# envoyproxy/ai-gateway

Hardware: AMD Instinct MI355X
Metric: req/sec (whole node) + p50 added latency, OpenAI chat/completions 4k-token body (higher is better)
Workload: dtype bf16; 1 GPU; model=aigw standalone: OpenAI /v1/chat/completions -> mock upstream (examples/basic), global_batch=128, seq_len=4096, parallelism=dp1, front=fast, cpu_affinity=numa node 1 (128 cpus)

## Files before the change

csrc/admission.hip:

```cpp

#include <hip/hip_runtime.h>

#include <atomic>
#include <cstdint>
#include <cstdio>
#include <cstring>
#include <mutex>
#include <vector>

#include "bpe_kernels.cuh"
#include "cache_kernels.cuh"

namespace aigw_fast {

namespace {

__global__ void excl_scan_kernel(const int32_t* __restrict__ in, int n,
                                 int32_t* __restrict__ excl,
                                 int32_t* __restrict__ total) {
  __shared__ int32_t wave_sum[4];
  __shared__ int32_t carry_s;
  if (threadIdx.x == 0) carry_s = 0;
  __syncthreads();
  int lane = (int)threadIdx.x & 63;
  int wave = (int)threadIdx.x >> 6;
  for (int base = 0; base < n; base += 256) {
    int i = base + (int)threadIdx.x;
    int32_t orig = (i < n) ? in[i] : 0;
    int32_t v = orig;
    for (int off = 1; off < 64; off <<= 1) {
      int32_t t = __shfl_up(v, off);
      if (lane >= off) v += t;
    }
    if (lane == 63) wave_sum[wave] = v;
    __syncthreads();
    int32_t wave_off = 0;
    for (int w = 0; w < wave; ++w) wave_off += wave_sum[w];
    if (i < n) excl[i] = carry_s + wave_off + v - orig;
    int32_t chunk_total =
        wave_sum[0] + wave_sum[1] + wave_sum[2] + wave_sum[3];
    __syncthreads();
    if (threadIdx.x == 0) carry_s += chunk_total;
    __syncthreads();
  }
  if (threadIdx.x == 0) *total = carry_s;
}

__global__ void f32_to_bf16_kernel(const float* __restrict__ in,
                                   bf16* __restrict__ out, int n) {
  int i = blockIdx.x * blockDim.x + threadIdx.x;
  if (i < n) out[i] = (bf16)in[i];
}

__global__ void tok_flags_kernel(const int32_t* __restrict__ out_ids, int n,
                                 uint8_t* __restrict__ flags) {
  int i = blockIdx.x * blockDim.x + threadIdx.x;
  if (i < n) flags[i] = out_ids[i] >= 0;
}

__global__ void meanpool_tokens_kernel(
    const int32_t* __restrict__ ids, const int32_t* __restrict__ ghead,
    const int32_t* __restrict__ req_excl, const int32_t* __restrict__ counts,
    int n_req, const bf16* __restrict__ emb, int dim, int P,
    float* __restrict__ out, int32_t* __restrict__ cnt) {
  constexpr int STAGE = 128;
  __shared__ int32_t tok_ids[STAGE];
  int r = blockIdx.x;
  int p = blockIdx.y;
  if (r >= n_req) return;
  int dim2 = dim >> 1;
  int col2 = threadIdx.x;
  int s = req_excl[r], c = counts[r];
  int chunk = (c + P - 1) / P;
  int j0 = p * chunk;
  int j1 = j0 + chunk;
  if (j1 > c) j1 = c;
  const uint32_t* emb2 = reinterpret_cast<const uint32_t*>(emb);
  float acc_lo = 0.f, acc_hi = 0.f;
  int n = 0;
  for (int base = j0; base < j1; base += STAGE) {
    if (threadIdx.x < STAGE && base + (int)threadIdx.x < j1)
      tok_ids[threadIdx.x] = ids[ghead[s + base + threadIdx.x]];
    __syncthreads();
    int here = j1 - base < STAGE ? j1 - base : STAGE;
    if (col2 < dim2) {
      for (int q = 0; q < here; ++q) {
        int tok = tok_ids[q];
        if (tok < 0) continue;
        uint32_t v = emb2[(long long)tok * dim2 + col2];
        bf16 lo, hi;
        uint16_t vlo = (uint16_t)(v & 0xffffu), vhi = (uint16_t)(v >> 16);
        memcpy(&lo, &vlo, 2);
        memcpy(&hi, &vhi, 2);
        acc_lo += __bfloat162float(lo);
        acc_hi += __bfloat162float(hi);
        ++n;
      }
    }
    __syncthreads();
  }
  if (col2 < dim2 && n) {
    atomicAdd(&out[(long long)r * dim + 2 * col2], acc_lo);
    atomicAdd(&out[(long long)r * dim + 2 * col2 + 1], acc_hi);
    if (col2 == 0) atomicAdd(&cnt[r], n);
  }
}

__global__ void park_pending_kernel(const bf16* __restrict__ q,
                                    const int32_t* __restrict__ slots,
                                    int n_req, int dim,
                                    bf16* __restrict__ pending) {
  int r = blockIdx.x;
  int col = threadIdx.x;
  if (r >= n_req || col >= dim) return;
  int slot = slots[r];
  if (slot < 0) return;
  pending[(size_t)slot * dim + col] = q[(size_t)r * dim + col];
}

__global__ void bf16_to_fp8_kernel(const bf16* __restrict__ in,
                                   uint8_t* __restrict__ out, int n) {
  int i = (blockIdx.x * blockDim.x + threadIdx.x) * 2;
  if (i >= n) return;
  float a = (float)in[i];
  float b = (i + 1 < n) ? (float)in[i + 1] : 0.f;
  int packed = __builtin_amdgcn_cvt_pk_fp8_f32(a, b, 0, false);
  out[i] = (uint8_t)(packed & 0xff);
  if (i + 1 < n) out[i + 1] = (uint8_t)((packed >> 8) & 0xff);
}

#define HIP_OK(expr)                                                   \
  do {                                                                 \
    hipError_t _e = (expr);                                            \
    if (_e != hipSuccess) {                                            \
      fprintf(stderr, "aigw admission: %s failed: %s\n", #expr,        \
              hipGetErrorString(_e));                                  \
      return false;                                                    \
    }                                                                  \
  } while (0)

}

class GpuAdmissionDirect {
 public:
  static constexpr int kSets = 2;

  struct BatchSet {
    hipStream_t stream{};
    hipEvent_t event{};
    char* h_bytes = nullptr;
    int64_t* h_off = nullptr;
    int32_t* h_counts = nullptr;
    unsigned long long* h_best = nullptr;
    int32_t* h_slots = nullptr;
    uint8_t* d_bytes = nullptr;
    int64_t* d_off = nullptr;
    uint8_t* d_flags = nullptr;
    uint8_t* d_gflags = nullptr;
    int32_t* d_blk = nullptr;
    int32_t* d_excl = nullptr;
    int32_t* d_totals = nullptr;
    int32_t* d_seg_start = nullptr;
    int32_t* d_seg_req = nullptr;
    int32_t* d_ghead = nullptr;
    int32_t* d_out_ids = nullptr;
    int32_t* d_counts = nullptr;
    int32_t* d_req_excl = nullptr;
    float* d_pool = nullptr;
    int32_t* d_poolcnt = nullptr;
    bf16* d_poolbf = nullptr;
    float* d_gout = nullptr;
    bf16* d_q = nullptr;
    uint8_t* d_q8 = nullptr;
    unsigned long long* d_best = nullptr;
    int32_t* d_slots = nullptr;
    long long rows_in_flight = 0;
  };

  bool init(const long long* htab_keys, const int32_t* htab_rank, int htab_n,
            size_t max_bytes, int max_req, int device) {
    int count = 0;
    if (hipGetDeviceCount(&count) != hipSuccess || count == 0) return false;
    device_ = device >= 0 && device < count ? device : 0;
    HIP_OK(hipSetDevice(device_));
    max_bytes_ = max_bytes;
    max_req_ = max_req;
    htab_mask_ = htab_n - 1;
    HIP_OK(hipMalloc(&d_htab_keys_, sizeof(long long) * htab_n));
    HIP_OK(hipMalloc(&d_htab_rank_, sizeof(int32_t) * htab_n));
    HIP_OK(hipMemcpy(d_htab_keys_, htab_keys, sizeof(long long) * htab_n,
                     hipMemcpyHostToDevice));
    HIP_OK(hipMemcpy(d_htab_rank_, htab_rank, sizeof(int32_t) * htab_n,
                     hipMemcpyHostToDevice));
    int max_blocks = (int)((max_bytes + 255) / 256);
    for (int s = 0; s < kSets; ++s) {
      BatchSet& b = sets_[s];
      HIP_OK(hipStreamCreateWithFlags(&b.stream, hipStreamNonBlocking));
      HIP_OK(hipEventCreateWithFlags(
          &b.event, hipEventDisableTiming | hipEventBlockingSync));
      HIP_OK(hipHostMalloc(&b.h_bytes, max_bytes, hipHostMallocDefault));
      HIP_OK(hipHostMalloc(&b.h_off, sizeof(int64_t) * (max_req + 1),
                           hipHostMallocDefault));
      HIP_OK(hipHostMalloc(&b.h_counts, sizeof(int32_t) * max_req,
                           hipHostMallocDefault));
      HIP_OK(hipMalloc(&b.d_bytes, max_bytes));
      HIP_OK(hipMalloc(&b.d_off, sizeof(int64_t) * (max_req + 1)));
      HIP_OK(hipMalloc(&b.d_flags, max_bytes));
      HIP_OK(hipMalloc(&b.d_gflags, max_bytes));
      HIP_OK(hipMalloc(&b.d_blk, sizeof(int32_t) * max_blocks));
      HIP_OK(hipMalloc(&b.d_excl, sizeof(int32_t) * max_blocks));
      HIP_OK(hipMalloc(&b.d_totals, sizeof(int32_t) * 2));
      HIP_OK(hipMalloc(&b.d_seg_start, sizeof(int32_t) * max_bytes));
      HIP_OK(hipMalloc(&b.d_seg_req, sizeof(int32_t) * max_bytes));
      HIP_OK(hipMalloc(&b.d_ghead, sizeof(int32_t) * max_bytes));
      HIP_OK(hipMalloc(&b.d_out_ids, sizeof(int32_t) * max_bytes));
      HIP_OK(hipMalloc(&b.d_counts, sizeof(int32_t) * max_req));
      HIP_OK(hipMalloc(&b.d_req_excl, sizeof(int32_t) * (max_req + 1)));
    }
    ready_ = true;
    return true;
  }

  bool count(const char* bytes, size_t n, const int64_t* offsets, int n_req,
             int32_t* counts_out) {
    if (!submit(0, bytes, n, offsets, n_req, nullptr)) return false;
    return wait_set(0, n_req, counts_out, nullptr, nullptr);
  }

  bool submit(int s, const char* bytes, size_t n, const int64_t* offsets,
              int n_req, const int32_t* pending_slots) {
    if (!ready_ || n == 0 || n_req == 0 || n > max_bytes_ || n_req > max_req_)
      return false;
    BatchSet& b = sets_[s];
    HIP_OK(hipSetDevice(device_));
    if (bytes != nullptr) memcpy(b.h_bytes, bytes, n);
    memcpy(b.h_off, offsets, sizeof(int64_t) * (size_t)n_req);
    hipStream_t st = b.stream;
    HIP_OK(hipMemcpyAsync(b.d_bytes, b.h_bytes, n, hipMemcpyHostToDevice, st));
    HIP_OK(hipMemcpyAsync(b.d_off, b.h_off, sizeof(int64_t) * (size_t)n_req,
                          hipMemcpyHostToDevice, st));
    int blocks = (int)((n + 255) / 256);
    hipLaunchKernelGGL(seg_flags_count_kernel, dim3(blocks), dim3(256), 0, st,
                       b.d_bytes, (int)n, b.d_off, n_req, b.d_flags, b.d_blk,
                       b.d_counts);
    hipLaunchKernelGGL(excl_scan_kernel, dim3(1), dim3(256), 0, st,
                       b.d_blk, blocks, b.d_excl, b.d_totals);
    hipLaunchKernelGGL(seg_write_kernel, dim3(blocks), dim3(256), 0, st,
                       b.d_flags, (int)n, b.d_excl, b.d_off, n_req,
                       b.d_seg_start, b.d_seg_req);
    hipLaunchKernelGGL(group_flags_count_kernel, dim3(blocks), dim3(256), 0,
                       st, b.d_seg_start, b.d_seg_req, b.d_totals, b.d_off,
                       (int)n, b.d_gflags, b.d_blk);
    hipLaunchKernelGGL(excl_scan_kernel, dim3(1), dim3(256), 0, st,
                       b.d_blk, blocks, b.d_excl, b.d_totals + 1);
    hipLaunchKernelGGL(flag_compact_write_kernel, dim3(blocks), dim3(256), 0,
                       st, b.d_gflags, (int)n, b.d_excl, b.d_ghead);
    bool want_cache = pending_slots != nullptr && cache_on_;
    if (want_cache)
      HIP_OK(hipMemsetAsync(b.d_out_ids, 0xFF, sizeof(int32_t) * n, st));
    long long group_bound = (long long)n / 32 + n_req + 1;
    constexpr int kBpeBlock = 512;
    constexpr int kGroupsPerBlock = kBpeBlock / 64;
    int blocks2 = (int)((group_bound + kGroupsPerBlock - 1) / kGroupsPerBlock);
    hipLaunchKernelGGL(bpe_encode_grouped_dev_kernel, dim3(blocks2),
                       dim3(kBpeBlock), 0, st, b.d_bytes, b.d_seg_start, b.d_seg_req,
                       b.d_totals, (int)n, b.d_ghead, b.d_totals + 1,
                       d_htab_keys_, d_htab_rank_, htab_mask_, b.d_out_ids,
                       b.d_counts);
    if (want_cache) {
      if (!submit_cache(b, n, n_req, pending_slots)) return false;
    }
    HIP_OK(hipMemcpyAsync(b.h_counts, b.d_counts, sizeof(int32_t) * n_req,
                          hipMemcpyDeviceToHost, st));
    HIP_OK(hipEventRecord(b.event, st));
    return true;
  }

  bool wait_set(int s, int n_req, int32_t* counts_out, int32_t* rows_out,
                float* scores_out) {
    BatchSet& b = sets_[s];
    HIP_OK(hipEventSynchronize(b.event));
    memcpy(counts_out, b.h_counts, sizeof(int32_t) * (size_t)n_req);
    if (rows_out != nullptr && scores_out != nullptr) {
      long long rows_now = b.rows_in_flight;
      for (int i = 0; i < n_req; ++i) {
        rows_out[i] = -1;
        scores_out[i] = 0.f;
        if (rows_now > 0) {
          unsigned long long u = b.h_best[i];
          unsigned hi = (unsigned)(u >> 32);
          unsigned bits = (hi >= 0x80000000u) ? (hi ^ 0x80000000u) : ~hi;
          float score;
          memcpy(&score, &bits, 4);
          if (score >= threshold_) {
            rows_out[i] = (int32_t)(u & 0xFFFFFFFFu);
            scores_out[i] = score;
          }
        }
      }
    }
    return true;
  }


  char* staging(int s) { return sets_[s].h_bytes; }

  bool init_cache(const uint16_t* emb, int vocab, const uint16_t* proj,
                  int dim, long long capacity, float threshold,
                  int pending_cap, bool fp8) {
    if (!ready_ || dim != 384) return false;
    HIP_OK(hipSetDevice(device_));
    dim_ = dim;
    cap_ = capacity;
    threshold_ = threshold;
    vocab_ = vocab;
    pending_cap_ = pending_cap;
    fp8_ = fp8;
    HIP_OK(hipMalloc(&d_emb_, sizeof(bf16) * (size_t)vocab * dim));
    HIP_OK(hipMemcpy(d_emb_, emb, sizeof(bf16) * (size_t)vocab * dim,
                     hipMemcpyHostToDevice));
    HIP_OK(hipMalloc(&d_proj_, sizeof(bf16) * (size_t)dim * dim));
    HIP_OK(hipMemcpy(d_proj_, proj, sizeof(bf16) * (size_t)dim * dim,
                     hipMemcpyHostToDevice));
    size_t elt = fp8 ? 1 : sizeof(bf16);
    HIP_OK(hipMalloc(&d_index_, elt * (size_t)capacity * dim));
    HIP_OK(hipMemset(d_index_, 0, elt * (size_t)capacity * dim));
    HIP_OK(hipMalloc(&d_pending_, sizeof(bf16) * (size_t)pending_cap * dim));
    HIP_OK(hipStreamCreateWithFlags(&insert_stream_, hipStreamNonBlocking));
    for (int s = 0; s < kSets; ++s) {
      BatchSet& b = sets_[s];
      HIP_OK(hipMalloc(&b.d_pool, sizeof(float) * (size_t)max_req_ * dim));
      HIP_OK(hipMalloc(&b.d_poolcnt, sizeof(int32_t) * max_req_));
      HIP_OK(hipMalloc(&b.d_poolbf, sizeof(bf16) * (size_t)max_req_ * dim));
      HIP_OK(hipMalloc(&b.d_gout, sizeof(float) * (size_t)max_req_ * dim));
      HIP_OK(hipMalloc(&b.d_q, sizeof(bf16) * (size_t)max_req_ * dim));
      if (fp8) HIP_OK(hipMalloc(&b.d_q8, (size_t)max_req_ * dim));
      HIP_OK(hipMalloc(&b.d_best, sizeof(unsigned long long) * max_req_));
      HIP_OK(hipHostMalloc(&b.h_best, sizeof(unsigned long long) * max_req_,
                           hipHostMallocDefault));
// ... 48 lines not shown
                       b.d_q, b.d_slots, n_req, dim, d_pending_);
    long long rows_now = rows_visible_.load(std::memory_order_acquire);
    b.rows_in_flight = rows_now;
    if (rows_now > 0) {
      HIP_OK(hipMemsetAsync(b.d_best, 0, sizeof(unsigned long long) * n_req, st));
      constexpr int ROWTILES = 16;
      long long blocks = (rows_now + 64 * ROWTILES - 1) / (64 * ROWTILES);
      if (fp8_) {
        hipLaunchKernelGGL(bf16_to_fp8_kernel,
                           dim3((n_req * dim / 2 + 255) / 256), dim3(256), 0,
                           st, b.d_q, b.d_q8, n_req * dim);
        constexpr size_t L8 = 128 * (12 * 32 + 16) + 128 * 8;
        (void)hipFuncSetAttribute(
            reinterpret_cast<const void*>(
                &cache_topk_fp8_lds_kernel_t<12, ROWTILES>),
            hipFuncAttributeMaxDynamicSharedMemorySize, 160 * 1024);
        for (int q0 = 0; q0 < n_req; q0 += 128) {
          int kq = (n_req - q0) < 128 ? (n_req - q0) : 128;
          hipLaunchKernelGGL((cache_topk_fp8_lds_kernel_t<12, ROWTILES>),
                             dim3((unsigned)blocks), dim3(256), L8, st,
                             (const uint8_t*)d_index_, rows_now,
                             b.d_q8 + (size_t)q0 * dim, kq, dim, b.d_best + q0);
        }
      } else {
        constexpr size_t L = 128 * (12 * 32 + 8) * sizeof(bf16) + 128 * 8;
        (void)hipFuncSetAttribute(
            reinterpret_cast<const void*>(&cache_topk_lds_kernel_t<12, ROWTILES>),
            hipFuncAttributeMaxDynamicSharedMemorySize, 160 * 1024);
        for (int q0 = 0; q0 < n_req; q0 += 128) {
          int kq = (n_req - q0) < 128 ? (n_req - q0) : 128;
          hipLaunchKernelGGL((cache_topk_lds_kernel_t<12, ROWTILES>),
                             dim3((unsigned)blocks), dim3(256), L, st,
                             (const bf16*)d_index_, rows_now,
                             b.d_q + (size_t)q0 * dim, kq, dim, b.d_best + q0);
        }
      }
      HIP_OK(hipMemcpyAsync(b.h_best, b.d_best,
                            sizeof(unsigned long long) * n_req,
                            hipMemcpyDeviceToHost, st));
    }
    return true;
  }

  bool count_lookup(const char* bytes, size_t n, const int64_t* offsets,
                    int n_req, int32_t* counts_out,
                    const int32_t* pending_slots, int32_t* rows_out,
                    float* scores_out) {
    if (!cache_on_) return false;
    if (!submit(0, bytes, n, offsets, n_req, pending_slots)) return false;
    return wait_set(0, n_req, counts_out, rows_out, scores_out);
  }

  long long cache_insert(int pending_slot) {
    if (!cache_on_ || pending_slot < 0 || pending_slot >= pending_cap_)
      return -1;
    long long row = head_;
    head_ = (head_ + 1) % cap_;
    if (fp8_) {
      hipLaunchKernelGGL(bf16_to_fp8_kernel, dim3((dim_ / 2 + 255) / 256),
                         dim3(256), 0, insert_stream_,
                         d_pending_ + (size_t)pending_slot * dim_,
                         (uint8_t*)d_index_ + (size_t)row * dim_, dim_);
      if (hipGetLastError() != hipSuccess) return -1;
    } else {
      hipError_t e = hipMemcpyAsync(
          (bf16*)d_index_ + (size_t)row * dim_,
          d_pending_ + (size_t)pending_slot * dim_, sizeof(bf16) * dim_,
          hipMemcpyDeviceToDevice, insert_stream_);
      if (e != hipSuccess) return -1;
    }
    long long vis = rows_visible_.load(std::memory_order_relaxed);
    long long want = row + 1 > vis ? row + 1 : vis;
    if (want > cap_) want = cap_;
    rows_visible_.store(want, std::memory_order_release);
    return row;
  }

  ~GpuAdmissionDirect() {
    if (!ready_) return;
    for (int s = 0; s < kSets; ++s) {
      BatchSet& b = sets_[s];
      (void)hipStreamDestroy(b.stream);
      (void)hipEventDestroy(b.event);
      (void)hipHostFree(b.h_bytes);
      (void)hipHostFree(b.h_off);
      (void)hipHostFree(b.h_counts);
      (void)hipHostFree(b.h_best);
      (void)hipHostFree(b.h_slots);
      for (void* p : {(void*)b.d_bytes, (void*)b.d_off, (void*)b.d_flags,
                      (void*)b.d_gflags, (void*)b.d_blk, (void*)b.d_excl,
                      (void*)b.d_totals, (void*)b.d_seg_start,
                      (void*)b.d_seg_req, (void*)b.d_ghead,
                      (void*)b.d_out_ids, (void*)b.d_counts, (void*)b.d_pool,
                      (void*)b.d_poolcnt, (void*)b.d_poolbf, (void*)b.d_gout,
                      (void*)b.d_q, (void*)b.d_q8, (void*)b.d_best,
                      (void*)b.d_slots})
        (void)hipFree(p);
    }
    if (cache_on_) {
      (void)hipStreamDestroy(insert_stream_);
      for (void* p : {(void*)d_emb_, (void*)d_proj_, (void*)d_index_,
                      (void*)d_pending_})
        (void)hipFree(p);
    }
    for (void* p : {(void*)d_htab_keys_, (void*)d_htab_rank_})
      (void)hipFree(p);
  }

  bool ready() const { return ready_; }

 private:
  bool ready_ = false;
  bool cache_on_ = false;
  int device_ = 0;
  int dim_ = 0;
  int vocab_ = 0;
  int pending_cap_ = 0;
  long long cap_ = 0;
  long long head_ = 0;
  std::atomic<long long> rows_visible_{0};
  float threshold_ = 0.f;
  bool fp8_ = false;
  bf16* d_emb_ = nullptr;
  bf16* d_proj_ = nullptr;
  void* d_index_ = nullptr;
  bf16* d_pending_ = nullptr;
  hipStream_t insert_stream_{};
  size_t max_bytes_ = 0;
  int max_req_ = 0;
  int htab_mask_ = 0;
  long long* d_htab_keys_ = nullptr;
  int32_t* d_htab_rank_ = nullptr;
  BatchSet sets_[kSets];
};

GpuAdmissionDirect* admission_create(const long long* htab_keys,
                                     const int32_t* htab_rank, int htab_n,
                                     size_t max_bytes, int max_req, int device) {
  auto* a = new GpuAdmissionDirect();
  if (!a->init(htab_keys, htab_rank, htab_n, max_bytes, max_req, device)) {
    delete a;
    return nullptr;
  }
  return a;
}

bool admission_count(GpuAdmissionDirect* a, const char* bytes, size_t n,
                     const int64_t* offsets, int n_req, int32_t* counts_out) {
  return a->count(bytes, n, offsets, n_req, counts_out);
}

void admission_destroy(GpuAdmissionDirect* a) { delete a; }

bool admission_init_cache(GpuAdmissionDirect* a, const uint16_t* emb, int vocab,
                          const uint16_t* proj, int dim, long long capacity,
                          float threshold, int pending_cap, bool fp8) {
  return a->init_cache(emb, vocab, proj, dim, capacity, threshold, pending_cap,
                       fp8);
}

bool admission_count_lookup(GpuAdmissionDirect* a, const char* bytes, size_t n,
                            const int64_t* offsets, int n_req,
                            int32_t* counts_out, const int32_t* pending_slots,
                            int32_t* rows_out, float* scores_out) {
  return a->count_lookup(bytes, n, offsets, n_req, counts_out, pending_slots,
                         rows_out, scores_out);
}

long long admission_cache_insert(GpuAdmissionDirect* a, int pending_slot) {
  return a->cache_insert(pending_slot);
}

bool admission_submit(GpuAdmissionDirect* a, int set, const char* bytes,
                      size_t n, const int64_t* offsets, int n_req,
                      const int32_t* pending_slots) {
  return a->submit(set, bytes, n, offsets, n_req, pending_slots);
}

bool admission_wait(GpuAdmissionDirect* a, int set, int n_req,
                    int32_t* counts_out, int32_t* rows_out,
                    float* scores_out) {
  return a->wait_set(set, n_req, counts_out, rows_out, scores_out);
}

char* admission_staging(GpuAdmissionDirect* a, int set) {
  return a->staging(set);
}

}
```

csrc/aigw_fast_module.cpp:

```cpp

#include <pybind11/pybind11.h>
#include <pybind11/stl.h>

#include <cstdint>
#include <stdexcept>
#include <string>
#include <vector>

#include "fastpath.h"

namespace py = pybind11;
using namespace aigw_fast;

namespace aigw_fast {

GpuAdmissionDirect* admission_create(const long long* htab_keys,
                                     const int32_t* htab_rank, int htab_n,
                                     size_t max_bytes, int max_req, int device);
bool admission_count(GpuAdmissionDirect* a, const char* bytes, size_t n,
                     const int64_t* offsets, int n_req, int32_t* counts_out);
void admission_destroy(GpuAdmissionDirect* a);
bool admission_init_cache(GpuAdmissionDirect* a, const uint16_t* emb, int vocab,
                          const uint16_t* proj, int dim, long long capacity,
                          float threshold, int pending_cap, bool fp8);
bool admission_count_lookup(GpuAdmissionDirect* a, const char* bytes, size_t n,
                            const int64_t* offsets, int n_req,
                            int32_t* counts_out, const int32_t* pending_slots,
                            int32_t* rows_out, float* scores_out);
long long admission_cache_insert(GpuAdmissionDirect* a, int pending_slot);

}

namespace {

class AdmissionProbe {
 public:
  AdmissionProbe(py::buffer htab_keys, py::buffer htab_rank, size_t max_bytes,
                 int max_req, int device)
      : max_bytes_(max_bytes), max_req_(max_req) {
    py::buffer_info ki = htab_keys.request();
    py::buffer_info ri = htab_rank.request();
    if (ki.itemsize != 8 || ri.itemsize != 4)
      throw std::runtime_error("htab_keys must be int64, htab_rank int32");
    if (ki.size != ri.size || ki.size <= 0 || (ki.size & (ki.size - 1)) != 0)
      throw std::runtime_error("htab arrays must share a power-of-two length");
    if (max_bytes == 0 || max_req <= 0)
      throw std::runtime_error("max_bytes and max_req must be positive");
    adm_ = admission_create(static_cast<const long long*>(ki.ptr),
                            static_cast<const int32_t*>(ri.ptr), (int)ki.size,
                            max_bytes, max_req, device);
    if (adm_ == nullptr) throw std::runtime_error("admission init failed");
  }
  AdmissionProbe(const AdmissionProbe&) = delete;
  AdmissionProbe& operator=(const AdmissionProbe&) = delete;
  ~AdmissionProbe() {
    if (adm_ != nullptr) admission_destroy(adm_);
  }

  void init_cache(py::buffer emb, py::buffer proj, long long capacity,
                  float threshold, int pending_cap, bool fp8) {
    constexpr int dim = 384;
    py::buffer_info ei = emb.request();
    py::buffer_info pi = proj.request();
    if (ei.itemsize != 2 || pi.itemsize != 2)
      throw std::runtime_error("emb/proj must be bf16 (uint16 view)");
    int vocab = (int)(ei.size / dim);
    if (vocab <= 0 || (long long)vocab * dim != ei.size ||
        pi.size != (long long)dim * dim)
      throw std::runtime_error("emb/proj shape mismatch");
    if (capacity <= 0 || pending_cap <= 0)
      throw std::runtime_error("capacity and pending_cap must be positive");
    if (cache_on_) throw std::runtime_error("cache already initialised");
    if (!admission_init_cache(adm_, static_cast<const uint16_t*>(ei.ptr), vocab,
                              static_cast<const uint16_t*>(pi.ptr), dim,
                              capacity, threshold, pending_cap, fp8))
      throw std::runtime_error("native cache init failed");
    pending_cap_ = pending_cap;
    cache_on_ = true;
  }

  std::vector<int32_t> count(const std::vector<std::string>& texts) {
    pack(texts);
    std::vector<int32_t> counts(texts.size(), 0);
    bool ok;
    {
      py::gil_scoped_release release;
      ok = admission_count(adm_, bytes_.data(), bytes_.size(), offs_.data(),
                           (int)texts.size(), counts.data());
    }
    if (!ok) throw std::runtime_error("admission_count failed");
    return counts;
  }

  py::tuple count_lookup(const std::vector<std::string>& texts) {
    if (!cache_on_) throw std::runtime_error("init_cache() first");
    if ((long long)texts.size() > pending_cap_)
      throw std::runtime_error("more texts than pending slots");
    pack(texts);
    size_t nt = texts.size();
    std::vector<int32_t> counts(nt, 0), rows(nt, -1), slots(nt);
    std::vector<float> scores(nt, 0.f);
    for (size_t i = 0; i < nt; ++i) slots[i] = (int32_t)i;
    bool ok;
    {
      py::gil_scoped_release release;
      ok = admission_count_lookup(adm_, bytes_.data(), bytes_.size(),
                                  offs_.data(), (int)nt, counts.data(),
                                  slots.data(), rows.data(), scores.data());
    }
    if (!ok) throw std::runtime_error("admission_count_lookup failed");
    return py::make_tuple(counts, rows, scores);
  }

  long long insert(int slot) {
    if (!cache_on_) throw std::runtime_error("init_cache() first");
    long long row = admission_cache_insert(adm_, slot);
    if (row < 0) throw std::runtime_error("cache insert failed");
    return row;
  }

 private:
  void pack(const std::vector<std::string>& texts) {
    if (texts.empty() || (long long)texts.size() > max_req_)
      throw std::runtime_error("text count out of range");
    bytes_.clear();
    offs_.clear();
    for (const auto& t : texts) {
      offs_.push_back((int64_t)bytes_.size());
      bytes_.append(t);
    }
    if (bytes_.empty() || bytes_.size() > max_bytes_)
      throw std::runtime_error("batch bytes out of range");
  }

  GpuAdmissionDirect* adm_ = nullptr;
  size_t max_bytes_;
  int max_req_;
  int pending_cap_ = 0;
  bool cache_on_ = false;
  std::string bytes_;
  std::vector<int64_t> offs_;
};

}

PYBIND11_MODULE(aigw_fast, m) {
  m.doc() = "aigw native data-plane fast path";

  py::class_<AdmissionProbe>(m, "AdmissionProbe")
      .def(py::init<py::buffer, py::buffer, size_t, int, int>(),
           py::arg("htab_keys"), py::arg("htab_rank"), py::arg("max_bytes"),
           py::arg("max_req"), py::arg("device") = 0)
      .def("init_cache", &AdmissionProbe::init_cache, py::arg("emb_u16"),
           py::arg("proj_u16"), py::arg("capacity"), py::arg("threshold"),
           py::arg("pending_cap"), py::arg("fp8"))
      .def("count", &AdmissionProbe::count, py::arg("texts"))
      .def("count_lookup", &AdmissionProbe::count_lookup, py::arg("texts"))
      .def("insert", &AdmissionProbe::insert, py::arg("slot"));

  py::class_<FastMock>(m, "FastMock")
      .def(py::init<>())
      .def("start", &FastMock::start, py::arg("host"), py::arg("response"))
      .def("stop", &FastMock::stop)
      .def("requests", &FastMock::requests);

  m.def(
      "run_load",
      [](const std::string& host, uint16_t port, const std::string& path,
         py::bytes body, int connections, int per_conn) {
        LoadResult r;
        {
          std::string b = body;
          py::gil_scoped_release release;
          r = run_load(host, port, path, b, connections, per_conn);
        }
        py::dict d;
        d["elapsed_s"] = r.elapsed_s;
        d["completed"] = r.completed;
        d["errors"] = r.errors;
        d["p50_ms"] = r.p50_ms;
        d["p99_ms"] = r.p99_ms;
        return d;
      },
      py::arg("host"), py::arg("port"), py::arg("path"), py::arg("body"),
      py::arg("connections"), py::arg("per_conn"),
      "closed-loop native load generator (threads, keep-alive)");

  m.def(
      "run_load_pool",
      [](const std::string& host, uint16_t port, const std::string& path,
         py::list bodies, int connections, int per_conn, bool capture_last) {
        std::vector<std::string> pool;
        for (auto b : bodies) pool.push_back(b.cast<py::bytes>());
        LoadResult r;
        {
          py::gil_scoped_release release;
          r = run_load_pool(host, port, path, pool, connections, per_conn,
                            capture_last);
        }
        py::dict d;
        d["elapsed_s"] = r.elapsed_s;
        d["completed"] = r.completed;
        d["errors"] = r.errors;
        d["p50_ms"] = r.p50_ms;
        d["p99_ms"] = r.p99_ms;
        if (capture_last) {
          py::list last;
          for (const auto& b : r.last_bodies) last.append(py::bytes(b));
          d["last_bodies"] = last;
        }
        return d;
      },
      py::arg("host"), py::arg("port"), py::arg("path"), py::arg("bodies"),
      py::arg("connections"), py::arg("per_conn"),
      py::arg("capture_last") = false,
      "run_load with a cycling body pool (semantic-cache hit mixes); "
      "capture_last also returns each connection's final response body");

  py::class_<FastServer>(m, "FastServer")
      .def(py::init<>())
      .def(
          "add_route",
          [](FastServer& s, const std::string& name, const std::string& model_match,
             int retries, bool has_costs, bool eligible, py::list backends) {
            FastRoute r;
            r.name = name;
            r.model_match = model_match;
            r.retries = retries;
            r.has_costs = has_costs;
            r.eligible = eligible;
            for (auto item : backends) {
              py::dict d = item.cast<py::dict>();
              FastBackend b;
              b.name = d["name"].cast<std::string>();
              b.host = d["host"].cast<std::string>();
              b.port = d["port"].cast<uint16_t>();
              if (d.contains("bearer")) b.bearer = d["bearer"].cast<std::string>();
              if (d.contains("api_key_file"))
                b.api_key_file = d["api_key_file"].cast<std::string>();
              if (d.contains("model_override"))
// ... 140 lines not shown
```

csrc/bpe_kernels.cuh:

```cuda
#pragma once

#include <hip/hip_runtime.h>

#include <climits>
#include <cstdint>

__device__ __forceinline__ int byte_class(uint8_t b) {
  if (b == ' ') return 0;
  if (b == '\t' || b == '\n' || b == '\r' || b == 0x0b || b == 0x0c) return 1;
  if (b >= '0' && b <= '9') return 2;
  if ((b >= 'A' && b <= 'Z') || (b >= 'a' && b <= 'z') || b >= 0x80) return 3;
  return 4;
}

__global__ void seg_flags_kernel(const uint8_t* __restrict__ bytes, int n,
                                 uint8_t* __restrict__ flags) {
  int i = blockIdx.x * blockDim.x + threadIdx.x;
  if (i >= n) return;
  uint8_t f;
  if (i == 0) {
    f = 1;
  } else {
    uint8_t b = bytes[i], p = bytes[i - 1];
    f = (b == ' ') || (byte_class(b) != byte_class(p) && p != ' ');
// ... 311 lines not shown

__global__ void group_head_flags_kernel(const int32_t* __restrict__ seg_start,
                                        const int32_t* __restrict__ seg_req,
                                        int n_segs,
                                        const int64_t* __restrict__ req_off,
                                        uint8_t* __restrict__ flags) {
  int i = blockIdx.x * blockDim.x + threadIdx.x;
  if (i >= n_segs) return;
  uint8_t f;
  if (i == 0 || seg_req[i] != seg_req[i - 1]) {
    f = 1;
  } else {
    long long off = req_off[seg_req[i]];
    f = ((seg_start[i] - off) >> 5) != ((seg_start[i - 1] - off) >> 5);
  }
  flags[i] = f;
}

__global__ void group_head_flags_dev_kernel(const int32_t* __restrict__ seg_start,
                                            const int32_t* __restrict__ seg_req,
                                            const int32_t* __restrict__ n_segs_dev,
                                            const int64_t* __restrict__ req_off,
                                            uint8_t* __restrict__ flags) {
  int i = blockIdx.x * blockDim.x + threadIdx.x;
  if (i >= *n_segs_dev) return;
  uint8_t f;
  if (i == 0 || seg_req[i] != seg_req[i - 1]) {
    f = 1;
  } else {
    long long off = req_off[seg_req[i]];
    f = ((seg_start[i] - off) >> 5) != ((seg_start[i - 1] - off) >> 5);
  }
  flags[i] = f;
}

__global__ void __launch_bounds__(256)
group_flags_count_kernel(const int32_t* __restrict__ seg_start,
                         const int32_t* __restrict__ seg_req,
                         const int32_t* __restrict__ n_segs_dev,
                         const int64_t* __restrict__ req_off, int n,
                         uint8_t* __restrict__ flags,
                         int32_t* __restrict__ blk_counts) {
  int i = blockIdx.x * 256 + threadIdx.x;
  bool f = false;
  if (i < n) {
    if (i < *n_segs_dev) {
      if (i == 0 || seg_req[i] != seg_req[i - 1]) {
        f = true;
      } else {
        long long off = req_off[seg_req[i]];
        f = ((seg_start[i] - off) >> 5) != ((seg_start[i - 1] - off) >> 5);
      }
    }
    flags[i] = f;
  }
  int cnt = block256_flag_count(f);
  if (threadIdx.x == 0) blk_counts[blockIdx.x] = cnt;
}

__global__ void flag_compact_write_kernel(const uint8_t* __restrict__ flags, int n,
                                          const int32_t* __restrict__ blk_excl,
                                          int32_t* __restrict__ out_idx) {
  __shared__ int wave_base[4];
  int i = blockIdx.x * blockDim.x + threadIdx.x;
  int lane = threadIdx.x & 63;
  int wave = threadIdx.x >> 6;
  bool f = (i < n) && flags[i];
  uint64_t ballot = __ballot(f);
  if (lane == 0) wave_base[wave] = __popcll(ballot);
  __syncthreads();
  if (threadIdx.x == 0) {
    int acc = 0;
    for (int w = 0; w < 4; ++w) {
      int c = wave_base[w];
      wave_base[w] = acc;
      acc += c;
    }
  }
  __syncthreads();
  if (!f) return;
  int pos_in_wave = __popcll(ballot & ((1ull << lane) - 1ull));
  out_idx[blk_excl[blockIdx.x] + wave_base[wave] + pos_in_wave] = i;
}
```

setup.py:

```python

import os

from setuptools import setup

os.environ.setdefault("PYTORCH_ROCM_ARCH", "gfx950")

import pybind11
from setuptools import Extension
from torch.utils.cpp_extension import BuildExtension, CUDAExtension

setup(
    name="aigw",
    version="0.1.0",
    packages=["aigw"],
    ext_modules=[
        CUDAExtension(
            name="aigw_hip",
            sources=["csrc/aigw_kernels.hip"],
            extra_compile_args={
                "cxx": ["-O3", "-std=c++17"],
                "nvcc": ["-O3", "-std=c++17", "--offload-arch=gfx950"],
            },
        ),
        Extension(
            name="aigw_native",
            sources=["csrc/aigw_native.cpp"],
            include_dirs=[pybind11.get_include()],
            extra_compile_args=["-O3", "-std=c++17"],
            language="c++",
        ),
        CUDAExtension(
            name="aigw_fast",
            sources=[
                "csrc/aigw_fast_module.cpp",
                "csrc/fastpath.cpp",
                "csrc/admission.hip",
            ],
            extra_compile_args={
                "cxx": ["-O3", "-std=c++17"],
                "nvcc": ["-O3", "-std=c++17", "--offload-arch=gfx950"],
            },
            extra_link_args=["-lpthread"],
        ),
    ],
    cmdclass={"build_ext": BuildExtension},
)
```

Baseline: 218,600 req/s.

## Fuse admission pre-tokenize kernels with last-block scans and single staged upload

Rewrites the GPU admission front end so each 256-thread block processes a 4096-byte granule instead of 256 bytes. The separate single-block exclusive-scan launches are folded into the flag/count kernels through a last-block-done ticket. Offsets and bytes now share one staging buffer, so a single H2D copy replaces two, with an optional zero-copy path that is off by default. This cuts kernel launches and per-batch overhead at the cost of atomic ticket synchronization and fewer, larger blocks. It also adds a pipelined count API and a build-flag hook.

```diff
diff --git a/csrc/admission.hip b/csrc/admission.hip
--- a/csrc/admission.hip
+++ b/csrc/admission.hip
@@ -10,6 +10,13 @@
 
 #include "bpe_kernels.cuh"
 #include "cache_kernels.cuh"
+
+#ifndef AIGW_ADM_FOLD_UPLOAD
+#define AIGW_ADM_FOLD_UPLOAD 0
+#endif
+#ifndef AIGW_ADM_FOLD_SCAN
+#define AIGW_ADM_FOLD_SCAN 1
+#endif
 
 namespace aigw_fast {
 
@@ -148,18 +155,20 @@
   struct BatchSet {
     hipStream_t stream{};
     hipEvent_t event{};
+    char* h_stage = nullptr;
+    uint8_t* d_stage = nullptr;
+    uint8_t* h_stage_dev = nullptr;
     char* h_bytes = nullptr;
-    int64_t* h_off = nullptr;
     int32_t* h_counts = nullptr;
     unsigned long long* h_best = nullptr;
     int32_t* h_slots = nullptr;
     uint8_t* d_bytes = nullptr;
-    int64_t* d_off = nullptr;
     uint8_t* d_flags = nullptr;
     uint8_t* d_gflags = nullptr;
     int32_t* d_blk = nullptr;
     int32_t* d_excl = nullptr;
     int32_t* d_totals = nullptr;
+    unsigned* d_tickets = nullptr;
     int32_t* d_seg_start = nullptr;
     int32_t* d_seg_req = nullptr;
     int32_t* d_ghead = nullptr;
@@ -193,29 +202,42 @@
     HIP_OK(hipMemcpy(d_htab_rank_, htab_rank, sizeof(int32_t) * htab_n,
                      hipMemcpyHostToDevice));
     int max_blocks = (int)((max_bytes + 255) / 256);
+    size_t padded = (max_bytes + kAdmGranule - 1) / kAdmGranule * kAdmGranule;
+    header_bytes_ = (sizeof(int64_t) * ((size_t)max_req + 1) + 255) / 256 * 256;
     for (int s = 0; s < kSets; ++s) {
       BatchSet& b = sets_[s];
       HIP_OK(hipStreamCreateWithFlags(&b.stream, hipStreamNonBlocking));
       HIP_OK(hipEventCreateWithFlags(
           &b.event, hipEventDisableTiming | hipEventBlockingSync));
-      HIP_OK(hipHostMalloc(&b.h_bytes, max_bytes, hipHostMallocDefault));
-      HIP_OK(hipHostMalloc(&b.h_off, sizeof(int64_t) * (max_req + 1),
+      HIP_OK(hipHostMalloc(&b.h_stage, header_bytes_ + padded,
                            hipHostMallocDefault));
+      b.h_bytes = b.h_stage + header_bytes_;
+      void* stage_dev = nullptr;
+      HIP_OK(hipHostGetDevicePointer(&stage_dev, b.h_stage, 0));
+      b.h_stage_dev = static_cast<uint8_t*>(stage_dev);
       HIP_OK(hipHostMalloc(&b.h_counts, sizeof(int32_t) * max_req,
                            hipHostMallocDefault));
-      HIP_OK(hipMalloc(&b.d_bytes, max_bytes));
-      HIP_OK(hipMalloc(&b.d_off, sizeof(int64_t) * (max_req + 1)));
-      HIP_OK(hipMalloc(&b.d_flags, max_bytes));
-      HIP_OK(hipMalloc(&b.d_gflags, max_bytes));
+      HIP_OK(hipMalloc(&b.d_stage, header_bytes_ + padded));
+      b.d_bytes = b.d_stage + header_bytes_;
+      HIP_OK(hipMalloc(&b.d_flags, padded));
+      HIP_OK(hipMalloc(&b.d_gflags, padded));
       HIP_OK(hipMalloc(&b.d_blk, sizeof(int32_t) * max_blocks));
       HIP_OK(hipMalloc(&b.d_excl, sizeof(int32_t) * max_blocks));
       HIP_OK(hipMalloc(&b.d_totals, sizeof(int32_t) * 2));
+      HIP_OK(hipMalloc(&b.d_tickets, 16));
+      HIP_OK(hipMemset(b.d_tickets, 0, 16));
       HIP_OK(hipMalloc(&b.d_seg_start, sizeof(int32_t) * max_bytes));
       HIP_OK(hipMalloc(&b.d_seg_req, sizeof(int32_t) * max_bytes));
       HIP_OK(hipMalloc(&b.d_ghead, sizeof(int32_t) * max_bytes));
       HIP_OK(hipMalloc(&b.d_out_ids, sizeof(int32_t) * max_bytes));
       HIP_OK(hipMalloc(&b.d_counts, sizeof(int32_t) * max_req));
       HIP_OK(hipMalloc(&b.d_req_excl, sizeof(int32_t) * (max_req + 1)));
+      HIP_OK(hipMemset(b.d_totals, 0, sizeof(int32_t) * 2));
+      HIP_OK(hipMemset(b.d_blk, 0, sizeof(int32_t) * max_blocks));
+      HIP_OK(hipMemset(b.d_excl, 0, sizeof(int32_t) * max_blocks));
+      HIP_OK(hipMemset(b.d_seg_start, 0, sizeof(int32_t) * max_bytes));
+      HIP_OK(hipMemset(b.d_seg_req, 0, sizeof(int32_t) * max_bytes));
+      HIP_OK(hipMemset(b.d_ghead, 0, sizeof(int32_t) * max_bytes));
     }
     ready_ = true;
     return true;
@@ -234,27 +256,50 @@
     BatchSet& b = sets_[s];
     HIP_OK(hipSetDevice(device_));
     if (bytes != nullptr) memcpy(b.h_bytes, bytes, n);
-    memcpy(b.h_off, offsets, sizeof(int64_t) * (size_t)n_req);
+    size_t off_bytes = sizeof(int64_t) * (size_t)n_req;
+    memcpy(b.h_bytes - off_bytes, offsets, off_bytes);
     hipStream_t st = b.stream;
-    HIP_OK(hipMemcpyAsync(b.d_bytes, b.h_bytes, n, hipMemcpyHostToDevice, st));
-    HIP_OK(hipMemcpyAsync(b.d_off, b.h_off, sizeof(int64_t) * (size_t)n_req,
-                          hipMemcpyHostToDevice, st));
-    int blocks = (int)((n + 255) / 256);
-    hipLaunchKernelGGL(seg_flags_count_kernel, dim3(blocks), dim3(256), 0, st,
-                       b.d_bytes, (int)n, b.d_off, n_req, b.d_flags, b.d_blk,
-                       b.d_counts);
-    hipLaunchKernelGGL(excl_scan_kernel, dim3(1), dim3(256), 0, st,
-                       b.d_blk, blocks, b.d_excl, b.d_totals);
-    hipLaunchKernelGGL(seg_write_kernel, dim3(blocks), dim3(256), 0, st,
-                       b.d_flags, (int)n, b.d_excl, b.d_off, n_req,
+    const int64_t* d_off =
+        reinterpret_cast<const int64_t*>(b.d_bytes - off_bytes);
+#if AIGW_ADM_FOLD_UPLOAD
+    const uint8_t* src = b.h_stage_dev + header_bytes_;
+    const int64_t* src_off = reinterpret_cast<const int64_t*>(src - off_bytes);
+    constexpr bool kCopyIn = true;
+#else
+    HIP_OK(hipMemcpyAsync(b.d_bytes - off_bytes, b.h_bytes - off_bytes,
+                          off_bytes + n, hipMemcpyHostToDevice, st));
+    const uint8_t* src = b.d_bytes;
+    const int64_t* src_off = d_off;
+    constexpr bool kCopyIn = false;
+#endif
+#if AIGW_ADM_FOLD_SCAN
+    unsigned* seg_ticket = b.d_tickets;
+    unsigned* grp_ticket = b.d_tickets + 1;
+#else
+    unsigned* seg_ticket = nullptr;
+    unsigned* grp_ticket = nullptr;
+#endif
+    int blocks = (int)((n + kAdmGranule - 1) / kAdmGranule);
+    hipLaunchKernelGGL(seg_front_kernel, dim3(blocks), dim3(256), 0, st, src,
+                       (int)n, src_off, n_req, kCopyIn, b.d_bytes,
+                       const_cast<int64_t*>(d_off), b.d_flags, b.d_blk,
+                       b.d_counts, seg_ticket, grp_ticket, b.d_excl,
+                       b.d_totals);
+    if (seg_ticket == nullptr)
+      hipLaunchKernelGGL(excl_scan_kernel, dim3(1), dim3(256), 0, st,
+                         b.d_blk, blocks, b.d_excl, b.d_totals);
+    hipLaunchKernelGGL(seg_write_g_kernel, dim3(blocks), dim3(256), 0, st,
+                       b.d_flags, (int)n, b.d_excl, d_off, n_req,
                        b.d_seg_start, b.d_seg_req);
-    hipLaunchKernelGGL(group_flags_count_kernel, dim3(blocks), dim3(256), 0,
-                       st, b.d_seg_start, b.d_seg_req, b.d_totals, b.d_off,
-                       (int)n, b.d_gflags, b.d_blk);
-    hipLaunchKernelGGL(excl_scan_kernel, dim3(1), dim3(256), 0, st,
-                       b.d_blk, blocks, b.d_excl, b.d_totals + 1);
-    hipLaunchKernelGGL(flag_compact_write_kernel, dim3(blocks), dim3(256), 0,
-                       st, b.d_gflags, (int)n, b.d_excl, b.d_ghead);
+    hipLaunchKernelGGL(group_front_kernel, dim3(blocks), dim3(256), 0, st,
+                       b.d_seg_start, b.d_seg_req, b.d_totals, d_off,
+                       (int)n, b.d_gflags, b.d_blk, grp_ticket, seg_ticket, b.d_excl,
+                       b.d_totals + 1);
+    if (grp_ticket == nullptr)
+      hipLaunchKernelGGL(excl_scan_kernel, dim3(1), dim3(256), 0, st,
+                         b.d_blk, blocks, b.d_excl, b.d_totals + 1);
+    hipLaunchKernelGGL(group_compact_g_kernel, dim3(blocks), dim3(256), 0, st,
+                       b.d_gflags, b.d_totals, (int)n, b.d_excl, b.d_ghead);
     bool want_cache = pending_slots != nullptr && cache_on_;
     if (want_cache)
       HIP_OK(hipMemsetAsync(b.d_out_ids, 0xFF, sizeof(int32_t) * n, st));
@@ -469,14 +514,14 @@
       BatchSet& b = sets_[s];
       (void)hipStreamDestroy(b.stream);
       (void)hipEventDestroy(b.event);
-      (void)hipHostFree(b.h_bytes);
-      (void)hipHostFree(b.h_off);
+      (void)hipHostFree(b.h_stage);
       (void)hipHostFree(b.h_counts);
       (void)hipHostFree(b.h_best);
       (void)hipHostFree(b.h_slots);
-      for (void* p : {(void*)b.d_bytes, (void*)b.d_off, (void*)b.d_flags,
+      for (void* p : {(void*)b.d_stage, (void*)b.d_flags,
                       (void*)b.d_gflags, (void*)b.d_blk, (void*)b.d_excl,
-                      (void*)b.d_totals, (void*)b.d_seg_start,
+                      (void*)b.d_totals, (void*)b.d_tickets,
+                      (void*)b.d_seg_start,
                       (void*)b.d_seg_req, (void*)b.d_ghead,
                       (void*)b.d_out_ids, (void*)b.d_counts, (void*)b.d_pool,
                       (void*)b.d_poolcnt, (void*)b.d_poolbf, (void*)b.d_gout,
@@ -514,6 +559,7 @@
   bf16* d_pending_ = nullptr;
   hipStream_t insert_stream_{};
   size_t max_bytes_ = 0;
+  size_t header_bytes_ = 0;
   int max_req_ = 0;
   int htab_mask_ = 0;
   long long* d_htab_keys_ = nullptr;
diff --git a/csrc/aigw_fast_module.cpp b/csrc/aigw_fast_module.cpp
--- a/csrc/aigw_fast_module.cpp
+++ b/csrc/aigw_fast_module.cpp
@@ -3,6 +3,7 @@
 #include <pybind11/stl.h>
 
 #include <cstdint>
+#include <cstring>
 #include <stdexcept>
 #include <string>
 #include <vector>
@@ -28,6 +29,12 @@
                             int32_t* counts_out, const int32_t* pending_slots,
                             int32_t* rows_out, float* scores_out);
 long long admission_cache_insert(GpuAdmissionDirect* a, int pending_slot);
+bool admission_submit(GpuAdmissionDirect* a, int set, const char* bytes,
+                      size_t n, const int64_t* offsets, int n_req,
+                      const int32_t* pending_slots);
+bool admission_wait(GpuAdmissionDirect* a, int set, int n_req,
+                    int32_t* counts_out, int32_t* rows_out, float* scores_out);
+char* admission_staging(GpuAdmissionDirect* a, int set);
 
 }
 
@@ -112,6 +119,58 @@
     return py::make_tuple(counts, rows, scores);
   }
 
+  std::vector<std::vector<int32_t>> count_pipelined(
+      const std::vector<std::vector<std::string>>& batches) {
+    for (const auto& texts : batches) {
+      if (texts.empty() || (long long)texts.size() > max_req_)
+        throw std::runtime_error("text count out of range");
+      size_t total = 0;
+      for (const auto& t : texts) total += t.size();
+      if (total == 0 || total > max_bytes_)
+        throw std::runtime_error("batch bytes out of range");
+    }
+    std::vector<std::vector<int32_t>> out(batches.size());
+    bool ok = true;
+    {
+      py::gil_scoped_release release;
+      long long in_flight[2] = {-1, -1};
+      std::vector<int64_t> offs;
+      auto wait = [&](int s) {
+        if (in_flight[s] < 0) return;
+        auto& counts = out[(size_t)in_flight[s]];
+        if (!admission_wait(adm_, s, (int)counts.size(), counts.data(),
+                            nullptr, nullptr))
+          ok = false;
+        in_flight[s] = -1;
+      };
+      for (size_t i = 0; i < batches.size() && ok; ++i) {
+        int s = (int)(i % 2);
+        wait(s);
+        if (!ok) break;
+        const auto& texts = batches[i];
+        char* staging = admission_staging(adm_, s);
+        offs.clear();
+        size_t n = 0;
+        for (const auto& t : texts) {
+          offs.push_back((int64_t)n);
+          memcpy(staging + n, t.data(), t.size());
+          n += t.size();
+        }
+        out[i].assign(texts.size(), 0);
+        if (!admission_submit(adm_, s, nullptr, n, offs.data(),
+                              (int)texts.size(), nullptr)) {
+          ok = false;
+          break;
+        }
+        in_flight[s] = (long long)i;
+      }
+      wait(0);
+      wait(1);
+    }
+    if (!ok) throw std::runtime_error("pipelined admission failed");
+    return out;
+  }
+
   long long insert(int slot) {
     if (!cache_on_) throw std::runtime_error("init_cache() first");
     long long row = admission_cache_insert(adm_, slot);
@@ -156,6 +215,8 @@
            py::arg("pending_cap"), py::arg("fp8"))
       .def("count", &AdmissionProbe::count, py::arg("texts"))
       .def("count_lookup", &AdmissionProbe::count_lookup, py::arg("texts"))
+      .def("count_pipelined", &AdmissionProbe::count_pipelined,
+           py::arg("batches"))
       .def("insert", &AdmissionProbe::insert, py::arg("slot"));
 
   py::class_<FastMock>(m, "FastMock")
diff --git a/csrc/bpe_kernels.cuh b/csrc/bpe_kernels.cuh
--- a/csrc/bpe_kernels.cuh
+++ b/csrc/bpe_kernels.cuh
@@ -417,3 +417,303 @@
   int pos_in_wave = __popcll(ballot & ((1ull << lane) - 1ull));
   out_idx[blk_excl[blockIdx.x] + wave_base[wave] + pos_in_wave] = i;
 }
+
+
+constexpr int kAdmGranule = 4096;
+
+__device__ __forceinline__ int block256_sum(int v) {
+  __shared__ int wave_part[4];
+  #pragma unroll
+  for (int off = 32; off > 0; off >>= 1) v += __shfl_xor(v, off);
+  __syncthreads();
+  if ((threadIdx.x & 63) == 0) wave_part[threadIdx.x >> 6] = v;
+  __syncthreads();
+  return wave_part[0] + wave_part[1] + wave_part[2] + wave_part[3];
+}
+
+__device__ __forceinline__ int block256_excl_scan(int v, int& total) {
+  __shared__ int wave_tot[4];
+  int lane = (int)threadIdx.x & 63;
+  int wave = (int)threadIdx.x >> 6;
+  int incl = v;
+  #pragma unroll
+  for (int off = 1; off < 64; off <<= 1) {
+    int t = __shfl_up(incl, off);
+    if (lane >= off) incl += t;
+  }
+  __syncthreads();
+  if (lane == 63) wave_tot[wave] = incl;
+  __syncthreads();
+  int wave_off = 0;
+  for (int w = 0; w < wave; ++w) wave_off += wave_tot[w];
+  total = wave_tot[0] + wave_tot[1] + wave_tot[2] + wave_tot[3];
+  return wave_off + incl - v;
+}
+
+__device__ __forceinline__ void publish_count_scan_if_last(
+    int cnt, int32_t* blk_counts, unsigned* ticket, int32_t* excl,
+    int32_t* total) {
+  __shared__ int is_last;
+  int tid = threadIdx.x;
+  if (ticket == nullptr) {
+    if (tid == 0) blk_counts[blockIdx.x] = cnt;
+    return;
+  }
+  if (tid == 0) {
+    __hip_atomic_store(&blk_counts[blockIdx.x], cnt, __ATOMIC_RELAXED,
+                       __HIP_MEMORY_SCOPE_AGENT);
+    asm volatile("s_waitcnt vmcnt(0)" ::: "memory");
+    unsigned t = __hip_atomic_fetch_add(ticket, 1u, __ATOMIC_RELAXED,
+                                        __HIP_MEMORY_SCOPE_AGENT);
+    is_last = (t == gridDim.x - 1u);
+  }
+  __syncthreads();
+  if (!is_last) return;
+  if (tid == 0) {
+    __builtin_amdgcn_fence(__ATOMIC_ACQUIRE, "agent");
+    asm volatile("s_waitcnt vmcnt(0)" ::: "memory");
+  }
+  __syncthreads();
+  int nblk = (int)gridDim.x;
+  int carry = 0;
+  for (int base = 0; base < nblk; base += 256) {
+    int i = base + tid;
+    int v = (i < nblk) ? __hip_atomic_load(&blk_counts[i], __ATOMIC_RELAXED,
+                                           __HIP_MEMORY_SCOPE_AGENT)
+                       : 0;
+    int chunk_total;
+    int e = block256_excl_scan(v, chunk_total);
+    if (i < nblk) excl[i] = carry + e;
+    carry += chunk_total;
+  }
+  if (tid == 0) *total = carry;
+}
+
+__global__ void __launch_bounds__(256)
+seg_front_kernel(const uint8_t* src, int n, const int64_t* src_off, int n_req,
+                 bool copy_in, uint8_t* dst_bytes, int64_t* dst_off,
+                 uint8_t* __restrict__ flags, int32_t* blk_counts,
+                 int32_t* __restrict__ req_counts, unsigned* ticket,
+                 unsigned* rearm, int32_t* excl, int32_t* total) {
+  __shared__ __attribute__((aligned(16))) uint8_t forced[kAdmGranule];
+  __shared__ uint8_t wave_last[4];
+  int tid = threadIdx.x;
+  int lane = tid & 63;
+  int wave = tid >> 6;
+  int base = blockIdx.x * kAdmGranule;
+  int end = min(base + kAdmGranule, n);
+  int my = base + tid * 16;
+  int last_vec = ((n - 1) >> 4) << 4;
+  uint4 raw = *reinterpret_cast<const uint4*>(src + min(my, last_vec));
+  uint8_t halo = src[max(base - 1, 0)];
+  long long my_off = src_off[min(tid, n_req - 1)];
+  if (tid >= n_req) my_off = -1;
+  reinterpret_cast<uint4*>(forced)[tid] = make_uint4(0, 0, 0, 0);
+  int gtid = blockIdx.x * 256 + tid;
+  int gstride = gridDim.x * 256;
+  for (int r = gtid; r < n_req; r += gstride) {
+    req_counts[r] = 0;
+    if (copy_in) dst_off[r] = src_off[r];
+  }
+  if (gtid == 0 && rearm != nullptr)
+    __hip_atomic_store(rearm, 0u, __ATOMIC_RELAXED, __HIP_MEMORY_SCOPE_AGENT);
+  __syncthreads();
+  if (n_req <= 256) {
+    if (my_off >= base && my_off < end) forced[my_off - base] = 1;
+  } else {
+    int lo = 0, len = n_req;
+    while (len > 0) {
+      int step = (len + 255) / 256;
+      int idx = lo + tid * step;
+      bool below = (tid * step < len) && src_off[idx] < base;
+      int c = block256_sum(below ? 1 : 0);
+      if (step == 1) { lo += c; break; }
+      if (c == 0) break;
+      int new_lo = lo + (c - 1) * step + 1;
+      int new_len = min(step - 1, lo + len - new_lo);
+      lo = new_lo;
+      len = new_len;
+    }
+    for (int r = lo + tid; r < n_req; r += 256) {
+      long long off = src_off[r];
+      if (off >= end) break;
+      if (off >= base) forced[off - base] = 1;
+    }
+  }
+  if (copy_in && my < n) *reinterpret_cast<uint4*>(dst_bytes + my) = raw;
+  uint8_t b[16];
+  {
+    uint32_t w[4] = {raw.x, raw.y, raw.z, raw.w};
+    #pragma unroll
+    for (int j = 0; j < 16; ++j) b[j] = (uint8_t)(w[j >> 2] >> ((j & 3) * 8));
+  }
+  int up = __shfl_up((int)b[15], 1);
+  if (lane == 63) wave_last[wave] = b[15];
+  __syncthreads();
+  uint8_t p = (uint8_t)up;
+  if (lane == 0) p = (wave == 0) ? halo : wave_last[wave - 1];
+  uint4 fm = reinterpret_cast<const uint4*>(forced)[tid];
+  uint32_t fw[4] = {fm.x, fm.y, fm.z, fm.w};
+  uint32_t ow[4] = {0, 0, 0, 0};
+  int cnt = 0;
+  #pragma unroll
+  for (int j = 0; j < 16; ++j) {
+    int i = my + j;
+    uint8_t c = b[j];
+    bool f = false;
+    if (i < n) {
+      f = (i == 0) || (c == ' ') ||
+          (byte_class(c) != byte_class(p) && p != ' ') ||
+          ((fw[j >> 2] >> ((j & 3) * 8)) & 0xffu);
+    }
+    if (f) {
+      ow[j >> 2] |= 1u << ((j & 3) * 8);
+      ++cnt;
+    }
+    p = c;
+  }
+  if (my < n)
+    *reinterpret_cast<uint4*>(flags + my) = make_uint4(ow[0], ow[1], ow[2], ow[3]);
+  cnt = block256_sum(cnt);
+  publish_count_scan_if_last(cnt, blk_counts, ticket, excl, total);
+}
+
+__device__ __forceinline__ int granule_lane_base(int lane_cnt, int blk_base) {
+  int total;
+  return blk_base + block256_excl_scan(lane_cnt, total);
+}
+
+__global__ void __launch_bounds__(256)
+seg_write_g_kernel(const uint8_t* __restrict__ flags, int n,
+                   const int32_t* __restrict__ blk_excl,
+                   const int64_t* __restrict__ req_off, int n_req,
+                   int32_t* __restrict__ seg_start,
+                   int32_t* __restrict__ seg_req) {
+  int my = blockIdx.x * kAdmGranule + threadIdx.x * 16;
+  uint4 fm = *reinterpret_cast<const uint4*>(flags + min(my, ((n - 1) >> 4) << 4));
+  if (my >= n) fm = make_uint4(0, 0, 0, 0);
+  int blk_base = blk_excl[blockIdx.x];
+  int base = blockIdx.x * kAdmGranule;
+  int last = min(base + kAdmGranule, n) - 1;
+  long long my_off = req_off[min((int)threadIdx.x, n_req - 1)];
+  if ((int)threadIdx.x >= n_req) my_off = LLONG_MAX;
+  uint32_t fw[4] = {fm.x, fm.y, fm.z, fm.w};
+  int cnt = 0;
+  #pragma unroll
+  for (int k = 0; k < 4; ++k) cnt += __popc(fw[k] & 0x01010101u);
+  int pos = granule_lane_base(cnt, blk_base);
+  int blk_lo = 0, blk_hi = 0;
+  if (n_req <= 256) {
+    int packed = block256_sum((my_off <= base ? 1 : 0) |
+                              (my_off <= last ? 1 << 16 : 0));
+    blk_lo = packed & 0xffff;
+    blk_hi = packed >> 16;
+  } else {
+    int hi_lo = n_req, hi_hi = n_req;
+    while (blk_lo < hi_lo || blk_hi < hi_hi) {
+      if (blk_lo < hi_lo) {
+        int mid = (blk_lo + hi_lo) >> 1;
+        if (req_off[mid] <= base) blk_lo = mid + 1; else hi_lo = mid;
+      }
+      if (blk_hi < hi_hi) {
+        int mid = (blk_hi + hi_hi) >> 1;
+        if (req_off[mid] <= last) blk_hi = mid + 1; else hi_hi = mid;
+      }
+    }
+  }
+  if (cnt == 0) return;
+  int lo = blk_lo, hi = blk_hi;
+  while (lo < hi) {
+    int mid = (lo + hi) >> 1;
+    if (req_off[mid] <= my) lo = mid + 1; else hi = mid;
+  }
+  long long next_off = (lo < blk_hi) ? req_off[lo] : LLONG_MAX;
+  #pragma unroll
+  for (int j = 0; j < 16; ++j) {
+    if (!((fw[j >> 2] >> ((j & 3) * 8)) & 1u)) continue;
+    int i = my + j;
+    while (i >= next_off) {
+      ++lo;
+      next_off = (lo < blk_hi) ? req_off[lo] : LLONG_MAX;
+    }
+    if ((unsigned)pos < (unsigned)n) {
+      seg_start[pos] = i;
+      seg_req[pos] = lo - 1;
+    }
+    ++pos;
+  }
+}
+
+__global__ void __launch_bounds__(256)
+group_front_kernel(const int32_t* __restrict__ seg_start,
+                   const int32_t* __restrict__ seg_req,
+                   const int32_t* __restrict__ n_segs_dev,
+                   const int64_t* __restrict__ req_off, int n,
+                   uint8_t* __restrict__ flags, int32_t* blk_counts,
+                   unsigned* ticket, unsigned* rearm, int32_t* excl,
+                   int32_t* total) {
+  int n_segs = min(*n_segs_dev, n);
+  int base = blockIdx.x * kAdmGranule;
+  if (blockIdx.x == 0 && threadIdx.x == 0 && rearm != nullptr)
+    __hip_atomic_store(rearm, 0u, __ATOMIC_RELAXED, __HIP_MEMORY_SCOPE_AGENT);
+  int cnt = 0;
+  if (base < n_segs) {
+    int rq[16], rqp[16], ss[16], ssp[16];
+    #pragma unroll
+    for (int k = 0; k < 16; ++k) {
+      int ic = min(base + k * 256 + (int)threadIdx.x, n_segs - 1);
+      int ip = max(ic - 1, 0);
+      rq[k] = seg_req[ic];
+      ss[k] = seg_start[ic];
+      rqp[k] = seg_req[ip];
+      ssp[k] = seg_start[ip];
+    }
+    long long off[16];
+    #pragma unroll
+    for (int k = 0; k < 16; ++k) off[k] = req_off[rq[k]];
+    #pragma unroll
+    for (int k = 0; k < 16; ++k) {
+      int i = base + k * 256 + (int)threadIdx.x;
+      if (i < n_segs) {
+        bool f = i == 0 || rq[k] != rqp[k] ||
+                 ((ss[k] - off[k]) >> 5) != ((ssp[k] - off[k]) >> 5);
+        flags[i] = f;
+        cnt += f;
+      }
+    }
+  }
+  cnt = block256_sum(cnt);
+  publish_count_scan_if_last(cnt, blk_counts, ticket, excl, total);
+}
+
+__global__ void __launch_bounds__(256)
+group_compact_g_kernel(const uint8_t* __restrict__ flags,
+                       const int32_t* __restrict__ n_dev, int cap,
+                       const int32_t* __restrict__ blk_excl,
+                       int32_t* __restrict__ out_idx) {
+  int n = min(*n_dev, cap);
+  int blk_base = blk_excl[blockIdx.x];
+  int my = blockIdx.x * kAdmGranule + threadIdx.x * 16;
+  uint4 fm = *reinterpret_cast<const uint4*>(flags + min(my, ((cap - 1) >> 4) << 4));
+  uint32_t fw[4] = {0, 0, 0, 0};
+  if (my < n) {
+    fw[0] = fm.x; fw[1] = fm.y; fw[2] = fm.z; fw[3] = fm.w;
+    int valid = n - my;
+    if (valid < 16) {
+      #pragma unroll
+      for (int j = 0; j < 16; ++j)
+        if (j >= valid) fw[j >> 2] &= ~(0xffu << ((j & 3) * 8));
+    }
+  }
+  int cnt = 0;
+  #pragma unroll
+  for (int k = 0; k < 4; ++k) cnt += __popc(fw[k] & 0x01010101u);
+  int pos = granule_lane_base(cnt, blk_base);
+  if (cnt == 0) return;
+  #pragma unroll
+  for (int j = 0; j < 16; ++j) {
+    if (!((fw[j >> 2] >> ((j & 3) * 8)) & 1u)) continue;
+    if ((unsigned)pos < (unsigned)cap) out_idx[pos] = my + j;
+    ++pos;
+  }
+}
diff --git a/setup.py b/setup.py
--- a/setup.py
+++ b/setup.py
@@ -8,6 +8,8 @@
 import pybind11
 from setuptools import Extension
 from torch.utils.cpp_extension import BuildExtension, CUDAExtension
+
+ADMISSION_FLAGS = os.environ.get("AIGW_ADMISSION_FLAGS", "").split()
 
 setup(
     name="aigw",
@@ -38,7 +40,8 @@
             ],
             extra_compile_args={
                 "cxx": ["-O3", "-std=c++17"],
-                "nvcc": ["-O3", "-std=c++17", "--offload-arch=gfx950"],
+                "nvcc": ["-O3", "-std=c++17", "--offload-arch=gfx950"]
+                + ADMISSION_FLAGS,
             },
             extra_link_args=["-lpthread"],
         ),
```

After: 214,600 req/s. 1.8% lower.
